# LCSL/nys-koop-lqr

Measured on AMD Instinct MI355X. Metric: Nyström-Koopman fits/sec (K_nm build + A,B,C solve), N=1e5 m=2000 d=384, higher is better.
Workload: dtype f64

## Files before the change

### nys_koop_lqr_amd/csrc/nk_chol_flow.hip

```cpp
#include <cstdio>
#include <cstdlib>

#include "nk_common.h"
#include "nk_panel_body.h"
#include "nk_potrf_body.h"

namespace nk {

namespace {

constexpr int FLOW_THREADS = 256;
constexpr int FLOW_HDR = 16;
constexpr int FLOW_POLL_LIMIT = 1 << 22;

struct FlowSys {
  double* P;
  int64_t ldp;
  int m, extra;
  double* Linv;
  double* pivlog;
  int* info;
  unsigned long long* piv;
  int* flags;
  int nblk;
// ... 232 lines not shown
        update_quarter(s, r0, r1, c0, c1, k - 1, wm, wn, l15, l4, Cd);
        store_quarter(s, r0, r1, c0, c1, wm, wn, l15, l4, Cd);
        local_sync();
      }
      if (wave == 0)
        flow_potrf(s.P + (int64_t)c0 * s.ldp + c0, s.ldp, c1 - c0, s.Linv + (size_t)k * CHOL_WS, s.info, s.piv,
                   s.pivlog ? s.pivlog + c0 : nullptr, k, lane);
      publish(s, k, k);
      __syncthreads();
    } else {
      if (k > 0) {
        Quarter C;
        load_quarter(s, r0, r1, c0, c1, wm, wn, l15, l4, C);
        bool ok = true;
        for (int j = 0; j < k && ok;) {
          const int J = wait_tiles(a, s, i, k, j, k, sh);
          if (J < 0) { ok = false; break; }
          for (; j < J; ++j) update_quarter(s, r0, r1, c0, c1, j, wm, wn, l15, l4, C);
        }
        if (!ok) continue;
        store_quarter(s, r0, r1, c0, c1, wm, wn, l15, l4, C);
        local_sync();
      }
      if (wait_tiles(a, s, k, -1, k, k + 1, sh) < 0) continue;
      panel_tile(a, s, r0, r1, k, wave, lane);
      publish(s, i, k);
      __syncthreads();
    }
  }
}

}

bool chol_flow_enabled() {
  const char* e = getenv("NYSKOOP_CHOL_FLOW");
  return !(e && e[0] == '0');
}

static int flow_test_giveup(const CholSys* sys, int nsys, int total) {
  const char* e = getenv("NYSKOOP_CHOL_FLOW_TEST_GIVEUP");
  if (!e || !e[0]) return -1;
  long ticket = -1, want_nsys = 0, want_extra = 0;
  if (sscanf(e, "%ld,%ld,%ld", &ticket, &want_nsys, &want_extra) < 1) return -1;
  if (want_nsys > 0 && want_nsys != nsys) return -1;
  if (want_extra > 0 && want_extra != sys[0].extra) return -1;
  return (ticket >= 0 && ticket < total) ? (int)ticket : -1;
}

int cholesky_flow_pair(nk_ctx* ctx, const CholSys* sys, int nsys) {
  constexpr int NB = CHOL_NB;
  NK_REQUIRE(nsys >= 1 && nsys <= 2, "cholesky_flow_pair: 1..2 systems");
  FlowArgs a;
  memset(&a, 0, sizeof(a));
  a.nsys = nsys;
  a.fix = chol_fix_enabled();
  size_t words = FLOW_HDR;
  for (int q = 0; q < nsys; ++q) {
    const CholSys& y = sys[q];
    FlowSys& s = a.s[q];
    s.P = y.P; s.ldp = y.ldp; s.m = y.m; s.extra = y.extra; s.Linv = y.Linv; s.pivlog = y.pivlog;
    s.info = ctx->d_info + info_base(ctx) + q;
    s.piv = ctx->d_piv + 2 * (info_base(ctx) + q);
    s.nblk = (y.m + NB - 1) / NB;
    s.nex = (y.extra + NB - 1) / NB;
    words += (size_t)(s.nblk + s.nex) * s.nblk;
    for (int c = 0; c < s.nblk; ++c) a.total += 1 + std::max(0, s.nblk - c - 2) + s.nex;
  }
  const int slot = info_base(ctx) / 2;
  if (ctx->flow_words[slot] < words) {
    if (ctx->d_flow[slot]) NK_HIP(hipFree(ctx->d_flow[slot]));
    ctx->d_flow[slot] = nullptr;
    ctx->flow_words[slot] = 0;
    NK_HIP(hipMalloc(reinterpret_cast<void**>(&ctx->d_flow[slot]), words * sizeof(int)));
    ctx->flow_words[slot] = words;
  }
  a.test_giveup = flow_test_giveup(sys, nsys, a.total);
  a.hdr = ctx->d_flow[slot];
  int* f = a.hdr + FLOW_HDR;
  for (int q = 0; q < nsys; ++q) {
    a.s[q].flags = f;
    f += (size_t)(a.s[q].nblk + a.s[q].nex) * a.s[q].nblk;
  }
  NK_HIP(hipMemsetAsync(a.hdr, 0, words * sizeof(int), ctx->stream));
  const int grid = std::max(1, std::min(a.total, ctx->num_cu / 2));
  hipLaunchKernelGGL(chol_flow_kernel, dim3((unsigned)grid), dim3(FLOW_THREADS), 0, ctx->stream, a);
  NK_HIP(hipGetLastError());
  count_event(CNT_CHOL_FLOW);
  return NK_OK;
}

}
```

### nys_koop_lqr_amd/csrc/nk_common.h

```cpp
#pragma once
#include <hip/hip_runtime.h>
#include <stdint.h>
#include <stddef.h>
#include <string>
#include <vector>

#include "nyskoop.h"
#include "nk_lockstep.h"
#include "nk_gemm_plan.h"
#include "nk_chain_plan.h"

namespace nk {

void set_error(const char* fmt, ...);

#define NK_HIP(call)                                                                         \
  do {                                                                                       \
    hipError_t e_ = (call);                                                                  \
    if (e_ != hipSuccess) {                                                                  \
      nk::set_error("%s failed: %s (%s:%d)", #call, hipGetErrorString(e_), __FILE__, __LINE__); \
      return e_ == hipErrorOutOfMemory ? NK_ERR_OOM : NK_ERR_HIP;                            \
    }                                                                                        \
  } while (0)

// ... 25 lines not shown
  size_t off;
};

}

enum {
  EV_FIT_BEGIN = 0,
  EV_STAGED = 1,
  EV_KMAT_DONE = 2,
  EV_GRAM_DONE = 3,
  EV_SOLVE_BEGIN = 4,
  EV_FIT_END = 5,
  EV_SQRT_BEGIN = 6,
  EV_SQRT_END = 7,
  EV_LANDMARKS = 8,
  EV_SQRT_PREPARED = 9,
  EV_SQRT_RESID = 10,
  EV_SQRT_SCALARS = 11,
  EV_FORK = 12,
  EV_YPREP_DONE = 13,
  EV_GEMM_T0 = 14,
  EV_GEMM_T1 = 15,
  EV_COUNT = 16
};

enum {
  HS_SCRATCH = 0,
  HS_SQRT_FLAG = 8,
  HS_SQRT_RESID_AT_FLAG = 9,
  HS_SQRT_RESID_LAST = 10,
  HS_SQRT_C = 12,
  HS_SQRT_SUMSQ = 13,
  HS_SQRT_TRACE = 14,
  HS_REFINE = 16,
  HS_COUNT = 64
};
enum {
  SQ_C = 0,
  SQ_SUMSQ = 1,
  SQ_TRACE = 2,
  SQ_LINV2 = 3,
  SQ_FLAG = 5,
  SQ_RESID_AT_FLAG = 6,
  SQ_RESID_LAST = 7,
  SQ_COUNT = 8
};

struct nk_member_state;
struct nk_ctx {
  int device = 0;
  hipStream_t stream = nullptr;
  hipStream_t stream_main = nullptr;
  hipStream_t stream_side = nullptr;
  hipStream_t stream_copy = nullptr;
  hipStream_t stream_prep = nullptr;
  nk::Arena arena;
  nk::Arena arena_side;
  nk::Arena* cur_arena = nullptr;
  hipStream_t stream_la[2] = {nullptr, nullptr};
  hipEvent_t ev_la[2][4] = {};
  int compute_f32 = 0;
  hipEvent_t ev_fork = nullptr, ev_join = nullptr, ev_chain = nullptr;
  int* d_info = nullptr;
  unsigned long long* d_piv = nullptr;
  unsigned long long* h_piv = nullptr;
  double* d_scalars = nullptr;
  double* h_scalars = nullptr;
  int* h_info = nullptr;
  double* d_zeros = nullptr;
  hipEvent_t ev[EV_COUNT];
  int num_cu = 256;
  int kmat_mode = 0;
  double refine_pivot = 0.0;
  int refine_steps = 2;
  int strict_spd = 0;
  hipEvent_t ev_ext = nullptr;
  hipEvent_t ev_up[8] = {};
  nk_group* group = nullptr;
  nk_member_state* gstate = nullptr;
  int* d_flow[2] = {nullptr, nullptr};
  size_t flow_words[2] = {0, 0};
  bool spline_defer_svd = false;
  bool chol_flow_off = false;
  double* h_stage = nullptr;
  size_t h_stage_bytes = 0;
};

enum { NK_MODEL_NYSTROM = 0, NK_MODEL_SPLINE = 1 };
struct nk_model {
  int device = 0;
  int32_t m = 0, d = 0, p = 0;
  int32_t ktype = 0;
  double sigma0 = 0.0;
  double jitter = 0.0;
  double* buf = nullptr;
  size_t bytes = 0;
  double *A = nullptr, *B = nullptr, *C = nullptr, *W = nullptr, *S = nullptr, *Sinv = nullptr, *Z = nullptr,
         *winv = nullptr;
  bool has_ops = false;
  int32_t kind = 0;
  hipEvent_t ev_fetch = nullptr;
};

namespace nk {

struct SideScope {
  nk_ctx* c;
  hipStream_t s0;
  Arena* a0;
  explicit SideScope(nk_ctx* ctx, hipStream_t s = nullptr) : c(ctx), s0(ctx->stream), a0(ctx->cur_arena) {
    c->stream = s ? s : c->stream_side;
    c->cur_arena = &c->arena_side;
  }
  ~SideScope() {
    c->stream = s0;
    c->cur_arena = a0;
  }
};

struct ChainOnly {
  nk_ctx* c;
  bool b0;
  explicit ChainOnly(nk_ctx* ctx) : c(ctx), b0(ctx->chol_flow_off) { c->chol_flow_off = true; }
  ~ChainOnly() { c->chol_flow_off = b0; }
};

inline int info_base(const nk_ctx* c) { return c->stream != c->stream_main ? 2 : 0; }

__device__ __forceinline__ double exp_nonpos_ca() {
  double ca = __longlong_as_double(0x3e5ade156a5dcb37LL);
  asm volatile("" : "+v"(ca));
  return ca;
}
__device__ __forceinline__ double exp_nonpos(double x, double ca_v) {
  const double k = __builtin_rint(x * __longlong_as_double(0x3ff71547652b82feLL));
  double r = __builtin_fma(__longlong_as_double((long long)0xbfe62e42fefa39efULL), k, x);
  r = __builtin_fma(__longlong_as_double((long long)0xbc7abc9e3b39803fULL), k, r);
  double p;
#define NK_EXP_STEP(c) asm("v_fma_f64 %0, %1, %2, %3" : "=v"(p) : "v"(r), "v"(p), "s"(c))
  asm("v_fma_f64 %0, %1, %2, %3" : "=v"(p) : "v"(r), "v"(ca_v), "s"(__longlong_as_double(0x3e928af3fca7ab0cLL)));
  NK_EXP_STEP(__longlong_as_double(0x3ec71dee623fde64LL));
  NK_EXP_STEP(__longlong_as_double(0x3efa01997c89e6b0LL));
  NK_EXP_STEP(__longlong_as_double(0x3f2a01a014761f6eLL));
  NK_EXP_STEP(__longlong_as_double(0x3f56c16c1852b7b0LL));
  NK_EXP_STEP(__longlong_as_double(0x3f81111111122322LL));
  NK_EXP_STEP(__longlong_as_double(0x3fa55555555502a1LL));
  NK_EXP_STEP(__longlong_as_double(0x3fc5555555555511LL));
  NK_EXP_STEP(__longlong_as_double(0x3fe000000000000bLL));
#undef NK_EXP_STEP
  p = __builtin_fma(r, p, 1.0);
  p = __builtin_fma(r, p, 1.0);
  return x < -1075.0 ? 0.0 : ldexp(p, (int)k);
}
__device__ __forceinline__ double exp_nonpos(double x) { return exp_nonpos(x, exp_nonpos_ca()); }

__host__ __device__ __forceinline__ double log_pos(double x) {
#pragma clang fp contract(off)
  const double ln2_hi = 6.93147180369123816490e-01, ln2_lo = 1.90821492927058770002e-10;
  const double Lg1 = 6.666666666666735130e-01, Lg2 = 3.999999999940941908e-01, Lg3 = 2.857142874366239149e-01,
               Lg4 = 2.222219843214978396e-01, Lg5 = 1.818357216161805012e-01, Lg6 = 1.531383769920937332e-01,
               Lg7 = 1.479819860511658591e-01;
  uint64_t bits;
  __builtin_memcpy(&bits, &x, 8);
  int32_t hx = (int32_t)(bits >> 32);
  int k = 0;
  if (hx < 0x00100000) {
    x *= 1.80143985094819840000e+16;
    k -= 54;
    __builtin_memcpy(&bits, &x, 8);
    hx = (int32_t)(bits >> 32);
  }
  k += (hx >> 20) - 1023;
  hx &= 0x000fffff;
  const int32_t i = (hx + 0x95f64) & 0x100000;
  bits = ((uint64_t)(uint32_t)(hx | (i ^ 0x3ff00000)) << 32) | (bits & 0xffffffffULL);
  __builtin_memcpy(&x, &bits, 8);
  k += i >> 20;
  const double f = x - 1.0;
  const double dk = (double)k;
  if ((0x000fffff & (2 + hx)) < 3) {
    if (f == 0.0) return k == 0 ? 0.0 : dk * ln2_hi + dk * ln2_lo;
    const double R = f * f * (0.5 - 0.33333333333333333 * f);
    return k == 0 ? f - R : dk * ln2_hi - ((R - dk * ln2_lo) - f);
  }
  const double s = f / (2.0 + f);
  const double z = s * s;
  const double w = z * z;
  const double t1 = w * (Lg2 + w * (Lg4 + w * Lg6));
  const double t2 = z * (Lg1 + w * (Lg3 + w * (Lg5 + w * Lg7)));
  const double R = t2 + t1;
  if (((hx - 0x6147a) | (0x6b851 - hx)) > 0) {
    const double hfsq = 0.5 * f * f;
    return k == 0 ? f - (hfsq - s * (hfsq + R)) : dk * ln2_hi - ((hfsq - (s * (hfsq + R) + dk * ln2_lo)) - f);
  }
  return k == 0 ? f - s * (f - R) : dk * ln2_hi - ((s * (f - R) - dk * ln2_lo) - f);
}
__host__ __device__ __forceinline__ double tps_value(double r2) {
#pragma clang fp contract(off)
  return r2 > 0.0 ? r2 * log_pos(sqrt(r2)) : 0.0;
}

nk_group* group_new(int device, int size);
void group_attach(nk_group* g, int slot, nk_ctx* c);
void group_detach(nk_ctx* c);
int group_enter(nk_ctx* c);
int group_leave(nk_ctx* c);
void group_stats(nk_ctx* c, uint64_t out[4]);
// ... 408 lines not shown
```

### nys_koop_lqr_amd/csrc/nk_fit.hip

```cpp
#include "nk_common.h"
#include "nk_tn.h"
#include "nk_api_internal.h"

#include <cmath>
#include <cstring>
#include <cstdlib>
#include <algorithm>
#include <initializer_list>

using namespace nk;

static inline size_t gram_block1(int m, int p) { return (((size_t)(2 * m + p) * (m + p)) + 1) & ~(size_t)1; }
static inline size_t gram_doubles(int m, int d, int p) { return gram_block1(m, p) + (size_t)(m + d) * m; }


static int select_rows(const char* who, const int64_t* row_ranges, int32_t n_ranges, int64_t n, std::vector<int64_t>* rng,
                       int64_t* n_eff) {
  if (row_ranges && n_ranges > 0) {
    for (int i = 0; i < n_ranges; ++i) {
      const int64_t b = row_ranges[2 * i], e = row_ranges[2 * i + 1];
      NK_REQUIRE(0 <= b && b <= e && e <= n, "%s: row range %d = [%lld,%lld) outside [0,%lld)", who, i, (long long)b,
                 (long long)e, (long long)n);
      if (e > b) { rng->push_back(b); rng->push_back(e); }
    }
// ... 45 lines not shown
      passes.back().push_back(Piece{b, len});
      used += len;
      b += len;
    }
  }
  return passes;
}

struct KernelBlocks {
  int ktype = 0;
  double sigma0 = 0.0;
  int d = 0, p = 0, m = 0;
  const double* winv = nullptr;
  bool gram_form = false;
  MatIn zi, zo;
  double *center = nullptr, *Rt = nullptr, *sqr = nullptr, *Zto = nullptr, *sqzo = nullptr, *Zti = nullptr, *sqzi = nullptr;
  int64_t ldt = 0, ldzt = 0;
  int64_t ldf = 0, off_out = 0;
  int copy_inputs(nk_ctx* ctx, const double* xs, int64_t ldx, int64_t len, double* Fo) const {
    if (p > 0) NK_TRY(launch_copy2d(ctx, xs + d, ldx, Fo + m, ldf, len, p));
    return NK_OK;
  }
  int piece(nk_ctx* ctx, const double* xs, int64_t ldx, const double* ys, int64_t ldy, int64_t len, double* Fo) const {
    if (gram_form && len >= 2) {
      NK_TRY(prep_rows(ctx, xs, ldx, len, d, winv, center, Rt, ldt, sqr));
      NK_TRY(launch_kmat_gram(ctx, ktype, Rt, ldt, sqr, len, Zti, ldzt, sqzi, m, d, sigma0, Fo, ldf));
      NK_TRY(prep_rows(ctx, ys, ldy, len, d, winv, center, Rt, ldt, sqr));
      NK_TRY(launch_kmat_gram(ctx, ktype, Rt, ldt, sqr, len, Zto, ldzt, sqzo, m, d, sigma0, Fo + off_out, ldf));
    } else {
      NK_TRY(launch_kmat(ctx, ktype, xs, ldx, len, zi.ptr, zi.ld, m, d, winv, sigma0, Fo, ldf));
      NK_TRY(launch_kmat(ctx, ktype, ys, ldy, len, zo.ptr, zo.ld, m, d, winv, sigma0, Fo + off_out, ldf));
    }
    return copy_inputs(ctx, xs, ldx, len, Fo);
  }
};

static void fill_gram_stats(nk_ctx* ctx, nk_fit_stats* stats, bool staged, bool gram_deferred, float ms_gram_kernel,
                            int gram_launches) {
  memset(stats, 0, sizeof(*stats));
  stats->ms_upload = staged ? ev_ms(ctx, EV_FIT_BEGIN, EV_STAGED) : 0.0;
  stats->ms_kmat = ev_ms(ctx, EV_STAGED, EV_KMAT_DONE);
  stats->ms_gram = ev_ms(ctx, EV_KMAT_DONE, EV_GRAM_DONE);
  if (gram_deferred) ms_gram_kernel = ev_ms(ctx, EV_GEMM_T0, EV_GEMM_T1);
  stats->ms_gram_kernel_avg = gram_launches ? ms_gram_kernel / gram_launches : 0.0;
  stats->gram_kernel_launches = gram_launches;
}

struct FitGuard {
  nk_model* m = nullptr;
  hipStream_t s[5] = {};
  int ns = 0;
  void arm(nk_model* mdl, std::initializer_list<hipStream_t> streams) {
    m = mdl;
    for (hipStream_t q : streams) s[ns++] = q;
  }
  ~FitGuard() {
    if (m) {
      for (int i = 0; i < ns; ++i) (void)hipStreamSynchronize(s[i]);
      nk_model_destroy(m);
    }
  }
};


enum { FIT_FULL = 0, FIT_GRAM = 1, FIT_SOLVE = 2 };

struct NystromFit {
  nk_ctx* ctx; const nk_kernel_desc* kd;
  const double* X; int64_t ldx; const double* Y; int64_t ldy; int64_t n; int32_t d, p;
  const int64_t* row_ranges; int32_t n_ranges;
  const double* Zin; int64_t ldzi; const double* Zout; int64_t ldzo; int32_t m;
  double gamma, jitter; nk_model** model; nk_fit_stats* stats; int mode; double* gram_io;
  HostTrace tr;
  std::vector<int64_t> rng;
  int64_t n_eff = 0;
  bool same_centers = false;
  int mp = 0;
  double gamma_n = 0.0;
  nk_model* mdl = nullptr;
  FitGuard guard;
  MatIn x, y, zi, zo;
  int host_passes = 1;
  double *Kmm = nullptr, *Kj = nullptr, *Kj_in = nullptr, *Kxo = nullptr;
  bool landmarks_aside = false;
  double *G1 = nullptr, *G2 = nullptr, *G3 = nullptr, *G4 = nullptr;
  int64_t ldd = 0;
  float ms_gram_kernel = 0.f;
  int gram_launches = 0;
  bool gram_deferred = false, timed = false;
  bool f32 = false, overlap_prep = false, multi_pass = false, pipelined = false;
  KernelBlocks kb;
  std::vector<std::vector<Piece>> passes;
  int64_t f_rows = 0, maxlen = 0, ldt32 = 0, ldzt32 = 0, ldy32 = 0;
  double *F = nullptr, *Rt2 = nullptr, *sqr2 = nullptr;
  float *F32 = nullptr, *Rt32 = nullptr, *sq32 = nullptr, *Zt32 = nullptr, *sqz32 = nullptr, *Y32 = nullptr;
  SqrtPlan splan;
  int it = 0;
  double resid = 0.0;
  double *Sinvt = nullptr, *T1t = nullptr, *X1 = nullptr;
  double *Gsave = nullptr, *V1 = nullptr, *Wc = nullptr, *Ct = nullptr;
  CholSys sys[2];
  int chol_failed[2] = {0, 0}, rank_sys[2] = {0, 0}, refined[2] = {0, 0};
  double piv_ratio[2] = {1.0, 1.0}, refine_ratio[2] = {0.0, 0.0};
  bool redo_products = false;

  int run();
  int validate(), stage_rows(), stage_landmarks(), landmark_matrices(), alloc_gram(), load_gram(), prepare_features(), run_passes();
  int upload_pass(size_t ip), pass_f32(size_t ip), pass_f64(size_t ip), blocks_overlapped(const Piece& pc, double* Fo);
  int return_gram();
  int queue_sqrt_prep(), assemble_and_factor(), queue_sqrt_side(), sqrt_products(), operator_products();
  int settle_factorisations(), refine(), settle_sqrt();
  void read_refinement(), write_stats();
};

int NystromFit::validate() {
  NK_TRY(check_ctx(ctx));
  tr.mark("check_ctx/arena_reset");
  NK_REQUIRE(kd && Zout, "nk_nystrom_fit: null argument");
  NK_REQUIRE(mode == FIT_SOLVE || (X && Y), "nk_nystrom_fit: null data pointer");
  NK_REQUIRE(mode == FIT_GRAM || model != nullptr, "nk_nystrom_fit: null model pointer");
  NK_REQUIRE(mode == FIT_FULL || gram_io != nullptr, "nk_nystrom_gram/solve: null accumulator");
  NK_REQUIRE(n > 0 && d > 0 && p >= 0 && m > 0, "nk_nystrom_fit: sizes must be positive (n=%lld d=%d p=%d m=%d)",
             (long long)n, d, p, m);
  NK_REQUIRE(mode == FIT_SOLVE || (ldx >= d + p && ldy >= d), "nk_nystrom_fit: leading dimension too small");
  NK_REQUIRE(ldzo >= d, "nk_nystrom_fit: leading dimension too small");
  NK_REQUIRE(std::isfinite(gamma) && std::isfinite(jitter), "nk_nystrom_fit: gamma/jitter not finite");
  NK_REQUIRE(kd->type != NK_KERNEL_TPS, "nk_nystrom_fit: the thin-plate spline has no Nystrom fit (nk_spline_fit)");
  if (model) *model = nullptr;
  NK_TRY(select_rows("nk_nystrom_fit", row_ranges, n_ranges, n, &rng, &n_eff));
  same_centers = (Zin == nullptr) || (Zin == Zout && ldzi == ldzo);
  mp = m + p;
  gamma_n = gamma * (double)n_eff;

  NK_TRY(model_alloc(ctx, m, d, p, &mdl));
  guard.arm(mdl, {ctx->stream_main, ctx->stream_side, ctx->stream_prep, ctx->stream_la[0], ctx->stream_la[1]});
  mdl->ktype = kd->type; mdl->sigma0 = kd->sigma0; mdl->jitter = jitter;
  tr.mark("validate + model_alloc");
  return NK_OK;
}

int NystromFit::stage_rows() {
  const char* e = getenv("NYSKOOP_HOST_PASSES");
  const int want = e ? atoi(e) : 6;
  if (want > 1 && rng.size() == 2 && !ctx_recording(ctx) && (double)n_eff * (2.0 * d + p) * 8.0 >= 64e6 &&
      !is_device_ptr(X) && !is_device_ptr(Y))
    host_passes = want > 8 ? 8 : want;
  if (host_passes > 1) {
    x.ld = (d + p + 1) & ~(int64_t)1;
    y.ld = (d + 1) & ~(int64_t)1;
    double *xd = nullptr, *yd = nullptr;
    NK_TRY(arena_alloc_t(ctx, (size_t)n * x.ld, &xd));
    NK_TRY(arena_alloc_t(ctx, (size_t)n * y.ld, &yd));
    x.ptr = xd; y.ptr = yd; x.staged = y.staged = true;
  } else {
    NK_TRY(stage_in(ctx, X, ldx, n, d + p, &x));
    NK_TRY(stage_in(ctx, Y, ldy, n, d, &y));
  }
  return gather_ranges(ctx, d, p, n_eff, &rng, &x, &y);
}

int NystromFit::stage_landmarks() {
  NK_TRY(stage_in(ctx, Zout, ldzo, m, d, &zo));
  if (same_centers) zi = zo; else NK_TRY(stage_in(ctx, Zin, ldzi, m, d, &zi));
  NK_TRY(launch_copy2d(ctx, zo.ptr, zo.ld, mdl->Z, d, m, d));
  NK_HIP(hipEventRecord(ctx->ev[EV_STAGED], ctx->stream));
  tr.mark("staging issued");
  return NK_OK;
}

int NystromFit::landmark_matrices() {
  NK_TRY(arena_alloc_t(ctx, (size_t)m * m, &Kmm));
  NK_TRY(arena_alloc_t(ctx, (size_t)m * m, &Kj));
  if (same_centers) {
    Kj_in = Kj;
    Kxo = Kmm;
  } else {
    NK_TRY(arena_alloc_t(ctx, (size_t)m * m, &Kj_in));
    NK_TRY(arena_alloc_t(ctx, (size_t)m * m, &Kxo));
  }
  {
    const char* la = getenv("NYSKOOP_LANDMARKS_ASIDE");
    landmarks_aside = mode == FIT_FULL && n_eff >= 20000 && m >= 1024 && !ctx_recording(ctx) && !(la && la[0] == '0');
  }
  hipStream_t s0 = ctx->stream;
  if (landmarks_aside) {
    NK_HIP(hipEventRecord(ctx->ev[EV_FORK], ctx->stream));
    ctx->stream = ctx->stream_prep;
    NK_HIP(hipStreamWaitEvent(ctx->stream, ctx->ev[EV_FORK], 0));
  }
  int rc_l = launch_kmat(ctx, kd->type, zo.ptr, zo.ld, m, zo.ptr, zo.ld, m, d, mdl->winv, kd->sigma0, Kmm, m);
  if (rc_l == NK_OK) rc_l = launch_copy2d(ctx, Kmm, m, Kj, m, m, m);
  if (rc_l == NK_OK) rc_l = launch_add_diag(ctx, Kj, m, m, jitter);
// ... 52 lines not shown
      NK_TRY(arena_alloc_t(ctx, (size_t)maxlen, &kb.sqr));
    }
    if (overlap_prep && !f32) {
      NK_TRY(arena_alloc_t(ctx, (size_t)d * kb.ldt, &Rt2));
      NK_TRY(arena_alloc_t(ctx, (size_t)maxlen, &sqr2));
    }
    NK_TRY(arena_alloc_t(ctx, (size_t)d * kb.ldzt, &kb.Zto));
    NK_TRY(arena_alloc_t(ctx, (size_t)m, &kb.sqzo));
    if (kd->type == NK_KERNEL_LINEAR) NK_TRY(launch_fill(ctx, kb.center, d, 1, d, 0.0));
    else NK_TRY(launch_colmean(ctx, zo.ptr, zo.ld, m, d, kb.center));
    NK_TRY(prep_rows(ctx, zo.ptr, zo.ld, m, d, mdl->winv, kb.center, kb.Zto, kb.ldzt, kb.sqzo));
    if (same_centers) {
      kb.Zti = kb.Zto; kb.sqzi = kb.sqzo;
    } else {
      NK_TRY(arena_alloc_t(ctx, (size_t)d * kb.ldzt, &kb.Zti));
      NK_TRY(arena_alloc_t(ctx, (size_t)m, &kb.sqzi));
      NK_TRY(prep_rows(ctx, zi.ptr, zi.ld, m, d, mdl->winv, kb.center, kb.Zti, kb.ldzt, kb.sqzi));
    }
  }
  F32 = reinterpret_cast<float*>(F);
  ldt32 = (maxlen + 3) & ~(int64_t)3; ldzt32 = (m + 3) & ~3; ldy32 = (d + 3) & ~3;
  if (f32) {
    NK_REQUIRE(same_centers, "fp32 engine: separate input landmarks are not supported");
    double* tmp = nullptr;
    NK_TRY(arena_alloc_t(ctx, ((size_t)d * ldt32 + 1) / 2 + 2, &tmp)); Rt32 = reinterpret_cast<float*>(tmp);
    NK_TRY(arena_alloc_t(ctx, ((size_t)maxlen + 1) / 2 + 2, &tmp)); sq32 = reinterpret_cast<float*>(tmp);
    NK_TRY(arena_alloc_t(ctx, ((size_t)d * ldzt32 + 1) / 2 + 2, &tmp)); Zt32 = reinterpret_cast<float*>(tmp);
    NK_TRY(arena_alloc_t(ctx, ((size_t)m + 1) / 2 + 2, &tmp)); sqz32 = reinterpret_cast<float*>(tmp);
    NK_TRY(arena_alloc_t(ctx, ((size_t)f_rows * ldy32 + 1) / 2 + 2, &tmp)); Y32 = reinterpret_cast<float*>(tmp);
    NK_TRY(prep_rows_f32(ctx, zo.ptr, zo.ld, m, d, mdl->winv, kb.center, Zt32, ldzt32, sqz32));
  }
  multi_pass = passes.size() > 1;
  pipelined = host_passes > 1;
  return NK_OK;
}

int NystromFit::upload_pass(size_t ip) {
  for (const Piece& pc : passes[ip]) {
    NK_HIP(hipMemcpy2DAsync(const_cast<double*>(x.ptr) + pc.b * x.ld, (size_t)x.ld * 8, X + pc.b * ldx, (size_t)ldx * 8,
                            (size_t)(d + p) * 8, (size_t)pc.len, hipMemcpyHostToDevice, ctx->stream_side));
    NK_HIP(hipMemcpy2DAsync(const_cast<double*>(y.ptr) + pc.b * y.ld, (size_t)y.ld * 8, Y + pc.b * ldy, (size_t)ldy * 8,
                            (size_t)d * 8, (size_t)pc.len, hipMemcpyHostToDevice, ctx->stream_side));
  }
  NK_HIP(hipEventRecord(ctx->ev_up[ip & 7], ctx->stream_side));
  return NK_OK;
}

int NystromFit::run_passes() {
  if (pipelined) {
    NK_HIP(hipEventRecord(ctx->ev[EV_FORK], ctx->stream));
    NK_HIP(hipStreamWaitEvent(ctx->stream_side, ctx->ev[EV_FORK], 0));
    NK_TRY(upload_pass(0));
  }
  for (size_t ip = 0; ip < passes.size(); ++ip) {
    if (pipelined) NK_HIP(hipStreamWaitEvent(ctx->stream, ctx->ev_up[ip & 7], 0));
    NK_TRY(f32 ? pass_f32(ip) : pass_f64(ip));
    if (pipelined && ip + 1 < passes.size()) NK_TRY(upload_pass(ip + 1));
  }
  return NK_OK;
}

int NystromFit::pass_f32(size_t ip) {
  const std::vector<Piece>& ps = passes[ip];
  const double beta = ip == 0 ? 0.0 : 1.0;
  const int64_t ldf = kb.ldf, off_out = kb.off_out;
  int64_t o32 = 0;
  for (const Piece& pc : ps) {
    const double* xs = x.ptr + pc.b * x.ld;
    const double* ys = y.ptr + pc.b * y.ld;
    NK_TRY(prep_rows_f32(ctx, xs, x.ld, pc.len, d, mdl->winv, kb.center, Rt32, ldt32, sq32));
    NK_TRY(launch_kmat_gram_f32(ctx, kd->type, Rt32, ldt32, sq32, pc.len, Zt32, ldzt32, sqz32, m, d, kd->sigma0,
                                F32 + o32 * ldf, ldf));
    NK_TRY(prep_rows_f32(ctx, ys, y.ld, pc.len, d, mdl->winv, kb.center, Rt32, ldt32, sq32));
    NK_TRY(launch_kmat_gram_f32(ctx, kd->type, Rt32, ldt32, sq32, pc.len, Zt32, ldzt32, sqz32, m, d, kd->sigma0,
                                F32 + o32 * ldf + off_out, ldf));
    if (p > 0) NK_TRY(launch_cvt_f64_f32(ctx, xs + d, x.ld, F32 + o32 * ldf + m, ldf, pc.len, p));
    NK_TRY(launch_cvt_f64_f32(ctx, ys, y.ld, Y32 + o32 * ldy32, ldy32, pc.len, d));
    o32 += pc.len;
  }
  if (ip == 0) {
    NK_HIP(hipEventRecord(ctx->ev[EV_KMAT_DONE], ctx->stream));
    tr.mark("kmat issued");
  }
  TnProblemF pf[4];
  pf[0].A = F32; pf[0].B = F32; pf[0].lda = pf[0].ldb = ldf; pf[0].M = pf[0].N = mp; pf[0].C = G1; pf[0].ldc = mp;
  pf[0].tri = TRI_UPPER_MIRROR;
  pf[1].A = F32 + off_out; pf[1].B = F32; pf[1].lda = pf[1].ldb = ldf; pf[1].M = m; pf[1].N = mp; pf[1].C = G2; pf[1].ldc = mp;
  pf[2].A = F32 + off_out; pf[2].B = F32 + off_out; pf[2].lda = pf[2].ldb = ldf; pf[2].M = pf[2].N = m; pf[2].C = G3;
  pf[2].ldc = m; pf[2].tri = TRI_UPPER_MIRROR;
  pf[3].A = Y32; pf[3].lda = ldy32; pf[3].M = d; pf[3].N = m; pf[3].C = G4; pf[3].ldc = m; pf[3].B = F32 + off_out;
  pf[3].ldb = ldf;
  for (int q = 0; q < 4; ++q) pf[q].beta = beta;
  float ms1 = 0.f;
  NK_TRY(launch_gemm_tn_f32_multi(ctx, pf, 4, o32, 0, timed ? &ms1 : nullptr, multi_pass));
  if (multi_pass) ms_gram_kernel += ms1; else gram_deferred = timed;
  gram_launches += 1;
  return NK_OK;
}

int NystromFit::blocks_overlapped(const Piece& pc, double* Fo) {
  const double* xs = x.ptr + pc.b * x.ld;
  const double* ys = y.ptr + pc.b * y.ld;
  NK_HIP(hipEventRecord(ctx->ev[EV_FORK], ctx->stream));
  {
    SideScope side(ctx);
    NK_HIP(hipStreamWaitEvent(ctx->stream, ctx->ev[EV_FORK], 0));
    NK_TRY(prep_rows(ctx, ys, y.ld, pc.len, d, mdl->winv, kb.center, Rt2, kb.ldt, sqr2));
    NK_HIP(hipEventRecord(ctx->ev[EV_YPREP_DONE], ctx->stream));
  }
  NK_TRY(prep_rows(ctx, xs, x.ld, pc.len, d, mdl->winv, kb.center, kb.Rt, kb.ldt, kb.sqr));
  NK_TRY(launch_kmat_gram(ctx, kd->type, kb.Rt, kb.ldt, kb.sqr, pc.len, kb.Zti, kb.ldzt, kb.sqzi, m, d, kd->sigma0, Fo, kb.ldf));
  NK_HIP(hipStreamWaitEvent(ctx->stream, ctx->ev[EV_YPREP_DONE], 0));
  NK_TRY(launch_kmat_gram(ctx, kd->type, Rt2, kb.ldt, sqr2, pc.len, kb.Zto, kb.ldzt, kb.sqzo, m, d, kd->sigma0,
                          Fo + kb.off_out, kb.ldf));
  return kb.copy_inputs(ctx, xs, x.ld, pc.len, Fo);
}

int NystromFit::pass_f64(size_t ip) {
  const std::vector<Piece>& ps = passes[ip];
  const double beta = ip == 0 ? 0.0 : 1.0;
  const int64_t ldf = kb.ldf, off_out = kb.off_out;
  int64_t o = 0;
  for (const Piece& pc : ps) {
    if (overlap_prep) NK_TRY(blocks_overlapped(pc, F + o * ldf));
    else NK_TRY(kb.piece(ctx, x.ptr + pc.b * x.ld, x.ld, y.ptr + pc.b * y.ld, y.ld, pc.len, F + o * ldf));
    o += pc.len;
  }
  const int64_t rows = o;
  if (ip == 0) {
    NK_HIP(hipEventRecord(ctx->ev[EV_KMAT_DONE], ctx->stream));
    tr.mark("kmat issued");
  }
  TnProblem pr[4];
  pr[0].A = F; pr[0].B = F; pr[0].lda = pr[0].ldb = ldf; pr[0].M = pr[0].N = mp; pr[0].C = G1; pr[0].ldc = mp;
  pr[0].tri = TRI_UPPER_MIRROR;
  pr[1].A = F + off_out; pr[1].B = F; pr[1].lda = pr[1].ldb = ldf; pr[1].M = m; pr[1].N = mp; pr[1].C = G2;
  pr[1].ldc = mp;
  pr[2].A = F + off_out; pr[2].B = F + off_out; pr[2].lda = pr[2].ldb = ldf; pr[2].M = pr[2].N = m; pr[2].C = G3;
  pr[2].ldc = m; pr[2].tri = TRI_UPPER_MIRROR;
  pr[3].A = y.ptr + ps[0].b * y.ld; pr[3].lda = y.ld; pr[3].M = d; pr[3].N = m; pr[3].C = G4; pr[3].ldc = m;
  pr[3].B = F + off_out; pr[3].ldb = ldf;
  for (int q = 0; q < 4; ++q) pr[q].beta = beta;
  const bool single = ps.size() == 1;
  const bool fast = tn_fast_ok(pr[0]) && tn_fast_ok(pr[1]) && tn_fast_ok(pr[2]);
  const bool fast_y = fast && tn_fast_ok(pr[3]);
  bool y_done = false;
  if (fast) {
    const int np = (single && fast_y) ? 4 : 3;
    float ms1 = 0.f;
    NK_TRY(launch_gemm_tn_multi(ctx, pr, np, rows, 0, (timed && !pipelined) ? &ms1 : nullptr, multi_pass));
    if (multi_pass) ms_gram_kernel += ms1; else gram_deferred = timed;
    gram_launches += 1;
    y_done = np == 4;
  } else {
    GemmOpts sym;
    sym.tri = TRI_UPPER_MIRROR;
    float t3[3] = {0.f, 0.f, 0.f};
    NK_TRY(launch_gemm(ctx, true, false, mp, mp, rows, 1.0, F, ldf, F, ldf, beta, G1, mp, sym, timed ? &t3[0] : nullptr));
    NK_TRY(launch_gemm(ctx, true, false, m, mp, rows, 1.0, F + off_out, ldf, F, ldf, beta, G2, mp, GemmOpts(),
                       timed ? &t3[1] : nullptr));
    NK_TRY(launch_gemm(ctx, true, false, m, m, rows, 1.0, F + off_out, ldf, F + off_out, ldf, beta, G3, m, sym,
                       timed ? &t3[2] : nullptr));
    ms_gram_kernel += t3[0] + t3[1] + t3[2];
    gram_launches += 3;
  }
  if (!y_done) {
    int64_t oo = 0;
    bool first = true;
    for (const Piece& pc : ps) {
      NK_TRY(launch_gemm(ctx, true, false, d, m, pc.len, 1.0, y.ptr + pc.b * y.ld, y.ld, F + oo * ldf + off_out, ldf,
                         (first && ip == 0) ? 0.0 : 1.0, G4, m));
      oo += pc.len;
      first = false;
    }
  }
  return NK_OK;
}

int NystromFit::return_gram() {
  NK_HIP(hipMemcpyAsync(gram_io, G1, gram_doubles(m, d, p) * sizeof(double),
                        is_device_ptr(gram_io) ? hipMemcpyDeviceToDevice : hipMemcpyDeviceToHost, ctx->stream));
  NK_HIP(hipStreamSynchronize(ctx->stream));
  if (stats) {
    fill_gram_stats(ctx, stats, x.staged || y.staged, gram_deferred, ms_gram_kernel, gram_launches);
    stats->ms_total = ev_ms(ctx, EV_FIT_BEGIN, EV_GRAM_DONE);
  }
  if (ctx->arena.chunks.size() > 1 || ctx->arena_side.chunks.size() > 1) NK_TRY(arena_reset(ctx));
  return NK_OK;
}


int NystromFit::sqrt_products() {
  NK_TRY(launch_transpose(ctx, mdl->Sinv, m, Sinvt, m, m, m));
  if (same_centers) {
    NK_TRY(launch_copy2d(ctx, mdl->S, m, T1t, m, m, m));
    NK_TRY(launch_axpby2d(ctx, -jitter, mdl->Sinv, m, 1.0, T1t, m, m, m));
  } else {
    NK_TRY(launch_transpose(ctx, Kxo, m, X1, m, m, m));
    NK_TRY(launch_gemm(ctx, true, false, m, m, m, 1.0, X1, m, mdl->Sinv, m, 0.0, T1t, m));
  }
  return NK_OK;
}

int NystromFit::queue_sqrt_prep() {
  SideScope prep(ctx, ctx->stream_prep);
  NK_HIP(hipStreamWaitEvent(ctx->stream, ctx->ev[EV_LANDMARKS], 0));
  splan.lambda_min_hint = jitter > 0.0 ? jitter : 0.0;
  if (mode == FIT_FULL && n_eff >= 20000 && m >= 1024) {
    static const double frac = getenv("NYSKOOP_PREP_PAUSE") ? atof(getenv("NYSKOOP_PREP_PAUSE")) : 0.0;
    const int nb = (m + CHOL_NB - 1) / CHOL_NB;
    if (frac < 1.0) {
      splan.pause_event = ctx->ev_fork;
      splan.pause_step = std::max(0, std::min(nb - 1, (int)(frac * nb)));
    }
  }
  NK_TRY(sqrtm_prepare(ctx, Kj, m, m, &splan));
  NK_HIP(hipEventRecord(ctx->ev[EV_SQRT_PREPARED], ctx->stream));
  return NK_OK;
}

int NystromFit::assemble_and_factor() {
  if (landmarks_aside) NK_HIP(hipStreamWaitEvent(ctx->stream, ctx->ev[EV_LANDMARKS], 0));
  NK_TRY(launch_axpby2d(ctx, gamma_n, Kj_in, m, 1.0, G1, mp, m, m));
  if (p > 0) NK_TRY(launch_add_diag(ctx, G1 + (int64_t)m * mp + m, mp, p, gamma_n));
  NK_TRY(launch_axpby2d(ctx, gamma_n, Kj, m, 1.0, G3, m, m, m));
  NK_TRY(arena_alloc_t(ctx, gram_doubles(m, d, p), &Gsave));
  NK_HIP(hipMemcpyAsync(Gsave, G1, gram_doubles(m, d, p) * sizeof(double), hipMemcpyDeviceToDevice, ctx->stream));
  double *Linv = nullptr, *Linv2 = nullptr, *pivlog = nullptr;
  const int nblk = (mp + CHOL_NB - 1) / CHOL_NB;
  NK_TRY(arena_alloc_t(ctx, (size_t)nblk * CHOL_WS, &Linv));
  NK_TRY(arena_alloc_t(ctx, (size_t)nblk * CHOL_WS, &Linv2));
  NK_TRY(arena_alloc_t(ctx, (size_t)m * m, &V1));
  NK_TRY(arena_alloc_t(ctx, (size_t)m * m, &Sinvt));
  NK_TRY(arena_alloc_t(ctx, (size_t)m * m, &T1t));
  NK_TRY(arena_alloc_t(ctx, (size_t)m * m, &X1));
  NK_TRY(arena_alloc_t(ctx, (size_t)m * ldd, &Wc));
  NK_TRY(arena_alloc_t(ctx, (size_t)m * ldd, &Ct));
  NK_TRY(arena_alloc_t(ctx, (size_t)mp + m + 4, &pivlog));
  sys[0].P = G1; sys[0].ldp = mp; sys[0].m = mp; sys[0].Linv = Linv; sys[0].extra = m;
  sys[1].P = G3; sys[1].ldp = m; sys[1].m = m; sys[1].Linv = Linv2; sys[1].extra = d;
  sys[0].pivlog = pivlog; sys[1].pivlog = pivlog + mp + (mp & 1);
  NK_TRY(cholesky_aug_pair_async(ctx, sys, 2));
  tr.mark("cholesky + solves issued");
  return NK_OK;
}

int NystromFit::queue_sqrt_side() {
  SideScope side(ctx);
  NK_HIP(hipStreamWaitEvent(ctx->stream, ctx->ev_fork, 0));
  NK_HIP(hipStreamWaitEvent(ctx->stream, ctx->ev[EV_SQRT_PREPARED], 0));
  NK_HIP(hipEventRecord(ctx->ev[EV_SQRT_BEGIN], ctx->stream));
  NK_TRY(sqrtm_finish(ctx, &splan, mdl->S, mdl->Sinv));
  NK_HIP(hipEventRecord(ctx->ev[EV_SQRT_END], ctx->stream));
  NK_TRY(sqrt_products());
  NK_HIP(hipEventRecord(ctx->ev_join, ctx->stream));
  return NK_OK;
}

int NystromFit::operator_products() {
  NK_TRY(launch_transpose(ctx, G2, mp, V1, m, m, m));
  NK_TRY(launch_gemm(ctx, true, false, m, m, m, 1.0, V1, m, T1t, m, 0.0, X1, m));
  NK_TRY(launch_gemm(ctx, true, false, m, m, m, 1.0, Sinvt, m, X1, m, 0.0, mdl->A, mp));
  if (p > 0) NK_TRY(launch_gemm(ctx, true, false, m, p, m, 1.0, Sinvt, m, G2 + m, mp, 0.0, mdl->B, mp));
  NK_TRY(launch_transpose(ctx, G4, m, Wc, ldd, d, m));
  NK_TRY(launch_gemm(ctx, true, false, m, d, m, 1.0, mdl->S, m, Wc, ldd, 0.0, Ct, ldd));
  NK_TRY(launch_transpose(ctx, Ct, ldd, mdl->C, m, m, d));
  NK_TRY(launch_gemm(ctx, true, false, d, mp, m, 1.0, Ct, ldd, mdl->A, mp, 0.0, mdl->W, mp));
  return NK_OK;
}

int NystromFit::settle_factorisations() {
  NK_TRY(cholesky_fail_flags(ctx, sys, 2, chol_failed, piv_ratio));
  tr.mark("final sync");
  bool chol_rerun = false;
  if (chol_failed[0] == CHOL_FLOW_GIVEUP || chol_failed[1] == CHOL_FLOW_GIVEUP) {
    ChainOnly chain(ctx);
    NK_HIP(hipMemcpyAsync(G1, Gsave, gram_doubles(m, d, p) * sizeof(double), hipMemcpyDeviceToDevice, ctx->stream));
    NK_TRY(cholesky_aug_pair_async(ctx, sys, 2));
    NK_TRY(cholesky_fail_flags(ctx, sys, 2, chol_failed, piv_ratio));
    chol_rerun = true;
  }
  rank_sys[0] = mp; rank_sys[1] = m;
  redo_products = chol_rerun;
  if (ctx->strict_spd == 2) chol_failed[0] = chol_failed[1] = -1;
  if (chol_failed[0] || chol_failed[1]) {
    if (ctx->strict_spd == 1) {
      set_error("Cholesky: system %d is numerically rank deficient (non-positive or rounding-level pivot; the reference's "
                "lstsq truncates here) and strict mode is on", chol_failed[0] ? 0 : 1);
      return NK_ERR_NOT_SPD;
    }
    const double rcond = 2.220446049250313e-16;
    for (int q = 0; q < 2; ++q) {
      if (!chol_failed[q]) continue;
      PinvInfo pi;
      if (q == 0)
        NK_TRY(pinv_right_divide(ctx, Gsave, mp, mp, Gsave + (size_t)mp * mp, mp, m, G2, mp, rcond, &pi));
      else
        NK_TRY(pinv_right_divide(ctx, Gsave + gram_block1(m, p), m, m, Gsave + gram_block1(m, p) + (size_t)m * m, m, d, G4,
                                 m, rcond, &pi));
      if (!pi.converged) {
        set_error("rank-revealing fallback: Jacobi SVD of system %d did not converge in %d sweeps", q, pi.sweeps);
        return NK_ERR_NO_CONVERGENCE;
      }
      rank_sys[q] = pi.rank;
    }
    count_event(CNT_RANK_TRUNCATED);
    redo_products = true;
  }
  return NK_OK;
}

int NystromFit::refine() {
  const double refine_below = ctx->refine_pivot;
  const int refine_steps = ctx->refine_steps;
  double* refine_state = nullptr;
  NK_TRY(arena_alloc_t(ctx, (size_t)8, &refine_state));
  for (int q = 0; q < 2 && refine_steps > 0; ++q) {
    if (chol_failed[q] || !(piv_ratio[q] > 0.0) || piv_ratio[q] >= refine_below) continue;
    const int mq = sys[q].m, nr = sys[q].extra;
    const size_t off = q == 0 ? 0 : gram_block1(m, p);
    const double* Pq = Gsave + off;
    const double* Rq = Gsave + off + (size_t)mq * mq;
    double* Xq = G1 + off + (size_t)mq * mq;
    const ArenaMark mk = arena_mark(ctx);
// ... 9 lines not shown
      NK_TRY(launch_transpose(ctx, Res, mq, ResT, ldt_, nr, mq));
      NK_TRY(cholesky_solve_pair(ctx, &cs, 1));
      NK_TRY(launch_transpose(ctx, ResT, ldt_, Res, mq, mq, nr));
      NK_TRY(launch_refine_apply(ctx, Res, mq, Xq, mq, nr, mq, step, refine_state + 4 * q, partial));
    }
    NK_HIP(hipMemcpyAsync(ctx->h_scalars + HS_REFINE + 4 * q, refine_state + 4 * q, 4 * sizeof(double), hipMemcpyDeviceToHost,
                          ctx->stream));
    arena_release(ctx, mk);
    refined[q] = -1;
    redo_products = true;
  }
  return NK_OK;
}

int NystromFit::settle_sqrt() {
  const int vr = sqrtm_verdict(ctx, &splan, &it, &resid);
  if (vr == NK_SQRT_RETRY && splan.flow_gave_up) {
    ChainOnly chain(ctx);
    SqrtPlan again;
    again.lambda_min_hint = splan.lambda_min_hint;
    NK_TRY(sqrtm_prepare(ctx, Kj, m, m, &again));
    NK_TRY(sqrtm_finish(ctx, &again, mdl->S, mdl->Sinv));
    NK_HIP(hipStreamSynchronize(ctx->stream));
    const int vr2 = sqrtm_verdict(ctx, &again, &it, &resid);
    if (vr2 == NK_SQRT_RETRY) {
      count_event(CNT_SQRT_RETRY);
      NK_TRY(sqrtm_spd_coupled(ctx, Kj, m, m, mdl->S, mdl->Sinv, &it, &resid));
    } else {
      NK_TRY(vr2);
    }
    NK_TRY(sqrt_products());
    redo_products = true;
  } else if (vr == NK_SQRT_RETRY) {
    count_event(CNT_SQRT_RETRY);
    NK_TRY(sqrtm_spd_coupled(ctx, Kj, m, m, mdl->S, mdl->Sinv, &it, &resid));
    NK_TRY(sqrt_products());
    redo_products = true;
  } else {
    NK_TRY(vr);
  }
  return NK_OK;
}

void NystromFit::read_refinement() {
  for (int q = 0; q < 2; ++q)
    if (refined[q] < 0) {
      refined[q] = (int)ctx->h_scalars[HS_REFINE + 4 * q + 2];
      refine_ratio[q] = ctx->h_scalars[HS_REFINE + 4 * q + 3];
    }
  if (refined[0] > 0 || refined[1] > 0) count_event(CNT_REFINED);
}

void NystromFit::write_stats() {
  fill_gram_stats(ctx, stats, x.staged || y.staged, gram_deferred, ms_gram_kernel, gram_launches);
  stats->ms_total = ev_ms(ctx, EV_FIT_BEGIN, EV_FIT_END);
  stats->ms_sqrt = ev_ms(ctx, EV_SQRT_BEGIN, EV_SQRT_END);
  stats->ms_solve = ev_ms(ctx, EV_SOLVE_BEGIN, EV_FIT_END);
  stats->sqrt_iters = it;
  stats->sqrt_residual = resid;
  const double ne = (double)n_eff;
  const double t128 = 128.0;
  auto tiles = [&](double v) { return std::ceil(v / t128); };
  const double tmp_ = tiles(mp), tm_ = tiles(m);
  stats->gram_flops = 2.0 * ne * t128 * t128 * (tmp_ * (tmp_ + 1) / 2 + tm_ * tmp_ + tm_ * (tm_ + 1) / 2) +
                      2.0 * ne * (double)d * m;
  stats->kmat_pairs = 2.0 * ne * m * d + (same_centers ? 1.0 : 3.0) * (double)m * m * d;
  stats->rank_inner = rank_sys[0];
  stats->rank_inner_rec = rank_sys[1];
  stats->pivot_ratio_inner = piv_ratio[0];
  stats->pivot_ratio_inner_rec = piv_ratio[1];
  stats->refined = refined[0] + 16 * refined[1];
  stats->refine_ratio_inner = refine_ratio[0];
  stats->refine_ratio_inner_rec = refine_ratio[1];
}


int NystromFit::run() {
  NK_TRY(validate());
  NK_HIP(hipEventRecord(ctx->ev[EV_FIT_BEGIN], ctx->stream));
  NK_TRY(make_winv(ctx, kd, d, mdl->winv));
  if (mode != FIT_SOLVE) NK_TRY(stage_rows());
  NK_TRY(stage_landmarks());
  if (mode != FIT_GRAM) NK_TRY(landmark_matrices());
  NK_TRY(alloc_gram());
  if (mode == FIT_SOLVE) {
    NK_TRY(load_gram());
  } else {
    NK_TRY(prepare_features());
    NK_TRY(run_passes());
  }
  NK_HIP(hipEventRecord(ctx->ev[EV_GRAM_DONE], ctx->stream));
  if (mode == FIT_GRAM) return return_gram();

  NK_HIP(hipEventRecord(ctx->ev_fork, ctx->stream));
  tr.mark("gram issued");
  NK_TRY(queue_sqrt_prep());
  NK_TRY(assemble_and_factor());
  NK_TRY(queue_sqrt_side());
  NK_HIP(hipStreamWaitEvent(ctx->stream, ctx->ev_join, 0));
  NK_HIP(hipEventRecord(ctx->ev[EV_SOLVE_BEGIN], ctx->stream));
  tr.mark("side stream joined (queued)");
  NK_TRY(operator_products());
  NK_HIP(hipEventRecord(ctx->ev[EV_FIT_END], ctx->stream));
  tr.mark("solve issued");

  NK_TRY(settle_factorisations());
  NK_TRY(refine());
  NK_TRY(settle_sqrt());
  if (redo_products) {
    NK_TRY(operator_products());
    NK_HIP(hipStreamSynchronize(ctx->stream));
  }
  read_refinement();
  mdl->has_ops = true;
  if (stats) write_stats();
  tr.mark("stats");
  if (ctx->arena.chunks.size() > 1 || ctx->arena_side.chunks.size() > 1) NK_TRY(arena_reset(ctx));
  guard.m = nullptr;
  *model = mdl;
  return NK_OK;
}

extern "C" {

int nk_nystrom_fit(nk_ctx* ctx, const nk_kernel_desc* kd, const double* X, int64_t ldx, const double* Y, int64_t ldy,
                   int64_t n, int32_t d, int32_t p, const int64_t* row_ranges, int32_t n_ranges, const double* Zin,
                   int64_t ldzi, const double* Zout, int64_t ldzo, int32_t m, double gamma, double jitter,
                   nk_model** model, nk_fit_stats* stats) {
  NK_REQUIRE(model != nullptr, "nk_nystrom_fit: null argument");
  NystromFit f{ctx, kd, X, ldx, Y, ldy, n, d, p, row_ranges, n_ranges, Zin, ldzi, Zout, ldzo, m, gamma, jitter, model, stats,
               FIT_FULL, nullptr};
  return f.run();
}

int nk_gram_doubles(int32_t m, int32_t d, int32_t p, int64_t* count) {
  NK_REQUIRE(count && m > 0 && d > 0 && p >= 0, "nk_gram_doubles: bad argument");
  *count = (int64_t)gram_doubles(m, d, p);
  return NK_OK;
}

int nk_nystrom_gram(nk_ctx* ctx, const nk_kernel_desc* kd, const double* X, int64_t ldx, const double* Y, int64_t ldy,
                    int64_t n, int32_t d, int32_t p, const int64_t* row_ranges, int32_t n_ranges, const double* Zin,
                    int64_t ldzi, const double* Zout, int64_t ldzo, int32_t m, double* gram, nk_fit_stats* stats) {
  NystromFit f{ctx, kd, X, ldx, Y, ldy, n, d, p, row_ranges, n_ranges, Zin, ldzi, Zout, ldzo, m, 0.0, 0.0, nullptr, stats,
               FIT_GRAM, gram};
  return f.run();
}

int nk_nystrom_solve(nk_ctx* ctx, const nk_kernel_desc* kd, const double* Zin, int64_t ldzi, const double* Zout,
                     int64_t ldzo, int32_t m, int32_t d, int32_t p, const double* gram, int64_t n_total, double gamma,
                     double jitter, nk_model** model, nk_fit_stats* stats) {
  NK_REQUIRE(model != nullptr, "nk_nystrom_solve: null argument");
  NystromFit f{ctx, kd, nullptr, 0, nullptr, 0, n_total, d, p, nullptr, 0, Zin, ldzi, Zout, ldzo, m, gamma, jitter, model, stats,
               FIT_SOLVE, const_cast<double*>(gram)};
  return f.run();
}

static constexpr double SPLINE_SVD_WINDOW_PER_ROW = 2.0;

int nk_spline_fit(nk_ctx* ctx, const double* X, int64_t ldx, const double* Y, int64_t ldy, int64_t n, int32_t d, int32_t p,
                  const int64_t* row_ranges, int32_t n_ranges, const double* centers, int64_t ldc, int32_t m, double gamma,
                  nk_model** model, nk_fit_stats* stats) {
  NK_TRY(check_ctx(ctx));
  NK_REQUIRE(X && Y && centers && model, "nk_spline_fit: null argument");
  NK_REQUIRE(n > 0 && d > 0 && p >= 0 && m > 0, "nk_spline_fit: sizes must be positive (n=%lld d=%d p=%d m=%d)",
             (long long)n, d, p, m);
  NK_REQUIRE(ldx >= d + p && ldy >= d && ldc >= d, "nk_spline_fit: leading dimension too small");
  NK_REQUIRE(std::isfinite(gamma), "nk_spline_fit: gamma not finite");
  *model = nullptr;
  std::vector<int64_t> rng;
  int64_t n_eff = 0;
  NK_TRY(select_rows("nk_spline_fit", row_ranges, n_ranges, n, &rng, &n_eff));
  const int mp = m + p;
  const double gamma_n = gamma * (double)n_eff;

  nk_model* mdl = nullptr;
  NK_TRY(model_alloc(ctx, m, d, p, &mdl, NK_MODEL_SPLINE));
  FitGuard guard;
  guard.arm(mdl, {ctx->stream_main, ctx->stream_side});
// ... 159 lines not shown
```

Baseline: 24.55.

## Issue sqrtm prep before gram passes and narrow Cholesky flow grid widths

Moves the sqrt-matrix preparation (which includes a Cholesky flow on Kj) ahead of the gram passes on the prep stream, so it overlaps the K_nm build instead of the later pause-based interleave. The first gram pass then waits on the prep event, which fences the GEMMs behind the factorization. A new context field caps the persistent chol_flow kernel's workgroup count: a quarter of the CUs for prep when the gram dominates, and three eighths for the main pair factorization, leaving CUs free for concurrent work. Risk: the ip==0 fence can serialize the gram behind the whole prep, and narrower grids slow each factorization.

```diff
diff --git a/nys_koop_lqr_amd/csrc/nk_chol_flow.hip b/nys_koop_lqr_amd/csrc/nk_chol_flow.hip
--- a/nys_koop_lqr_amd/csrc/nk_chol_flow.hip
+++ b/nys_koop_lqr_amd/csrc/nk_chol_flow.hip
@@ -338,7 +338,8 @@
     f += (size_t)(a.s[q].nblk + a.s[q].nex) * a.s[q].nblk;
   }
   NK_HIP(hipMemsetAsync(a.hdr, 0, words * sizeof(int), ctx->stream));
-  const int grid = std::max(1, std::min(a.total, ctx->num_cu / 2));
+  const int width = ctx->chol_flow_wgs > 0 ? ctx->chol_flow_wgs : ctx->num_cu / 2;
+  const int grid = std::max(1, std::min(a.total, width));
   hipLaunchKernelGGL(chol_flow_kernel, dim3((unsigned)grid), dim3(FLOW_THREADS), 0, ctx->stream, a);
   NK_HIP(hipGetLastError());
   count_event(CNT_CHOL_FLOW);
diff --git a/nys_koop_lqr_amd/csrc/nk_common.h b/nys_koop_lqr_amd/csrc/nk_common.h
--- a/nys_koop_lqr_amd/csrc/nk_common.h
+++ b/nys_koop_lqr_amd/csrc/nk_common.h
@@ -131,6 +131,7 @@
   size_t flow_words[2] = {0, 0};
   bool spline_defer_svd = false;
   bool chol_flow_off = false;
+  int chol_flow_wgs = 0;
   double* h_stage = nullptr;
   size_t h_stage_bytes = 0;
 };
@@ -172,6 +173,13 @@
   bool b0;
   explicit ChainOnly(nk_ctx* ctx) : c(ctx), b0(ctx->chol_flow_off) { c->chol_flow_off = true; }
   ~ChainOnly() { c->chol_flow_off = b0; }
+};
+
+struct FlowWidth {
+  nk_ctx* c;
+  int w0;
+  FlowWidth(nk_ctx* ctx, int wgs) : c(ctx), w0(ctx->chol_flow_wgs) { c->chol_flow_wgs = wgs; }
+  ~FlowWidth() { c->chol_flow_wgs = w0; }
 };
 
 inline int info_base(const nk_ctx* c) { return c->stream != c->stream_main ? 2 : 0; }
diff --git a/nys_koop_lqr_amd/csrc/nk_fit.hip b/nys_koop_lqr_amd/csrc/nk_fit.hip
--- a/nys_koop_lqr_amd/csrc/nk_fit.hip
+++ b/nys_koop_lqr_amd/csrc/nk_fit.hip
@@ -151,7 +151,7 @@
   MatIn x, y, zi, zo;
   int host_passes = 1;
   double *Kmm = nullptr, *Kj = nullptr, *Kj_in = nullptr, *Kxo = nullptr;
-  bool landmarks_aside = false;
+  bool landmarks_aside = false, sqrt_early = false;
   double *G1 = nullptr, *G2 = nullptr, *G3 = nullptr, *G4 = nullptr;
   int64_t ldd = 0;
   float ms_gram_kernel = 0.f;
@@ -177,6 +177,8 @@
   int validate(), stage_rows(), stage_landmarks(), landmark_matrices(), alloc_gram(), load_gram(), prepare_features(), run_passes();
   int upload_pass(size_t ip), pass_f32(size_t ip), pass_f64(size_t ip), blocks_overlapped(const Piece& pc, double* Fo);
   int return_gram();
+  bool sqrt_factor_early() const;
+  int fence_sqrt_factor(size_t ip);
   int queue_sqrt_prep(), assemble_and_factor(), queue_sqrt_side(), sqrt_products(), operator_products();
   int settle_factorisations(), refine(), settle_sqrt();
   void read_refinement(), write_stats();
@@ -395,6 +397,7 @@
     NK_HIP(hipEventRecord(ctx->ev[EV_KMAT_DONE], ctx->stream));
     tr.mark("kmat issued");
   }
+  NK_TRY(fence_sqrt_factor(ip));
   TnProblemF pf[4];
   pf[0].A = F32; pf[0].B = F32; pf[0].lda = pf[0].ldb = ldf; pf[0].M = pf[0].N = mp; pf[0].C = G1; pf[0].ldc = mp;
   pf[0].tri = TRI_UPPER_MIRROR;
@@ -444,6 +447,7 @@
     NK_HIP(hipEventRecord(ctx->ev[EV_KMAT_DONE], ctx->stream));
     tr.mark("kmat issued");
   }
+  NK_TRY(fence_sqrt_factor(ip));
   TnProblem pr[4];
   pr[0].A = F; pr[0].B = F; pr[0].lda = pr[0].ldb = ldf; pr[0].M = pr[0].N = mp; pr[0].C = G1; pr[0].ldc = mp;
   pr[0].tri = TRI_UPPER_MIRROR;
@@ -515,18 +519,33 @@
   return NK_OK;
 }
 
+bool NystromFit::sqrt_factor_early() const {
+  if (mode != FIT_FULL || n_eff < 20000 || m < 1024 || ctx_recording(ctx)) return false;
+  if (ctx->chol_flow_off || !chol_flow_enabled()) return false;
+  const char* e = getenv("NYSKOOP_PREP_PAUSE");
+  return !(e && e[0]);
+}
+
+int NystromFit::fence_sqrt_factor(size_t ip) {
+  if (sqrt_early && ip == 0) NK_HIP(hipStreamWaitEvent(ctx->stream, ctx->ev[EV_SQRT_PREPARED], 0));
+  return NK_OK;
+}
+
 int NystromFit::queue_sqrt_prep() {
   SideScope prep(ctx, ctx->stream_prep);
   NK_HIP(hipStreamWaitEvent(ctx->stream, ctx->ev[EV_LANDMARKS], 0));
   splan.lambda_min_hint = jitter > 0.0 ? jitter : 0.0;
-  if (mode == FIT_FULL && n_eff >= 20000 && m >= 1024) {
-    static const double frac = getenv("NYSKOOP_PREP_PAUSE") ? atof(getenv("NYSKOOP_PREP_PAUSE")) : 0.0;
+  if (!sqrt_early && mode == FIT_FULL && n_eff >= 20000 && m >= 1024) {
+    const char* e = getenv("NYSKOOP_PREP_PAUSE");
+    const double frac = e ? atof(e) : 0.0;
     const int nb = (m + CHOL_NB - 1) / CHOL_NB;
     if (frac < 1.0) {
       splan.pause_event = ctx->ev_fork;
       splan.pause_step = std::max(0, std::min(nb - 1, (int)(frac * nb)));
     }
   }
+  const bool narrow = sqrt_early && (double)n_eff * d >= 9.0 * (double)m * m;
+  FlowWidth width(ctx, narrow ? std::max(1, ctx->num_cu / 4) : 0);
   NK_TRY(sqrtm_prepare(ctx, Kj, m, m, &splan));
   NK_HIP(hipEventRecord(ctx->ev[EV_SQRT_PREPARED], ctx->stream));
   return NK_OK;
@@ -553,6 +572,7 @@
   sys[0].P = G1; sys[0].ldp = mp; sys[0].m = mp; sys[0].Linv = Linv; sys[0].extra = m;
   sys[1].P = G3; sys[1].ldp = m; sys[1].m = m; sys[1].Linv = Linv2; sys[1].extra = d;
   sys[0].pivlog = pivlog; sys[1].pivlog = pivlog + mp + (mp & 1);
+  FlowWidth width(ctx, sqrt_early ? std::max(1, 3 * ctx->num_cu / 8) : 0);
   NK_TRY(cholesky_aug_pair_async(ctx, sys, 2));
   tr.mark("cholesky + solves issued");
   return NK_OK;
@@ -728,6 +748,8 @@
   if (mode != FIT_SOLVE) NK_TRY(stage_rows());
   NK_TRY(stage_landmarks());
   if (mode != FIT_GRAM) NK_TRY(landmark_matrices());
+  sqrt_early = sqrt_factor_early();
+  if (sqrt_early) NK_TRY(queue_sqrt_prep());
   NK_TRY(alloc_gram());
   if (mode == FIT_SOLVE) {
     NK_TRY(load_gram());
@@ -740,7 +762,7 @@
 
   NK_HIP(hipEventRecord(ctx->ev_fork, ctx->stream));
   tr.mark("gram issued");
-  NK_TRY(queue_sqrt_prep());
+  if (!sqrt_early) NK_TRY(queue_sqrt_prep());
   NK_TRY(assemble_and_factor());
   NK_TRY(queue_sqrt_side());
   NK_HIP(hipStreamWaitEvent(ctx->stream, ctx->ev_join, 0));
```

Result: faster. 24.97 (median of 6 runs) (+1.7%).
